# google-research/big_vision

Measured on NVIDIA H100. Metric: siglip_vit_b16_pairs_per_sec, higher is better.
Workload: dtype bf16

## Files before the change

big_vision_b200/csrc/attention.cu:

```cuda
#include "common.cuh"
#include "host_utils.h"
#include "kernels.h"

namespace bv {

namespace {

constexpr int T = 64;
constexpr int BOX_BYTES = T * 64 * 2;
constexpr float LOG2E = 1.4426950408889634f;
constexpr float LN2 = 0.6931471805599453f;
constexpr int THREADS = 128;

template <int DH>
struct Geo {
  static_assert(DH == 64 || DH == 72 || DH == 80 || DH == 96 || DH == 104, "head dims 64, 72, 80, 96, 104");
  static constexpr int TILE_BYTES = DH > 64 ? 2 * BOX_BYTES : BOX_BYTES;
  static constexpr int KSTEPS = (DH + 15) / 16;
  static_assert(KSTEPS >= 4 && KSTEPS <= 8, "one or two 64-column boxes");
  static constexpr int R = DH / 2;
  static constexpr int FWD_SMEM = 5 * TILE_BYTES + 1024 + 64;
  static constexpr int BWD_SMEM = 6 * TILE_BYTES + 1024 + 64;
};

__device__ __forceinline__ float ex2(float x) {
  float y;
  asm("ex2.approx.ftz.f32 %0, %1;" : "=f"(y) : "f"(x));
  return y;
}

int make_tmap_bnd(CUtensorMap* m, const void* ptr, int dh, int H, int64_t N, int64_t B, int64_t ld, int64_t bs) {
  if (dh == 64) {
    uint64_t dims[3] = {static_cast<uint64_t>(H) * 64, static_cast<uint64_t>(N), static_cast<uint64_t>(B)};
    uint64_t strides[2] = {static_cast<uint64_t>(ld) * 2, static_cast<uint64_t>(bs) * 2};
    uint32_t box[3] = {64, T, 1};
    return make_tmap(m, CU_TENSOR_MAP_DATA_TYPE_BFLOAT16, 3, ptr, dims, strides, box, true);
  }
  uint64_t dims[4] = {static_cast<uint64_t>(dh), static_cast<uint64_t>(H), static_cast<uint64_t>(N),
                      static_cast<uint64_t>(B)};
  uint64_t strides[3] = {static_cast<uint64_t>(dh) * 2, static_cast<uint64_t>(ld) * 2, static_cast<uint64_t>(bs) * 2};
  uint32_t box[4] = {64, 1, T, 1};
  return make_tmap(m, CU_TENSOR_MAP_DATA_TYPE_BFLOAT16, 4, ptr, dims, strides, box, true);
}

template <int DH>
__device__ __forceinline__ void load_tile(uint32_t dst, const CUtensorMap* m, uint32_t bar, int h, int row, int b) {
  if constexpr (DH == 64) {
    tma_load_3d(dst, m, bar, h * DH, row, b);
  } else {
    tma_load_4d(dst, m, bar, 0, h, row, b);
    tma_load_4d(dst + BOX_BYTES, m, bar, 64, h, row, b);
  }
}

__device__ __forceinline__ uint64_t desc_k(uint32_t tile) { return wgmma_desc_sw128(tile, 16u, 1024u); }
__device__ __forceinline__ uint64_t desc_mn(uint32_t tile) { return wgmma_desc_sw128(tile, 8192u, 1024u); }
constexpr uint64_t KSTEP_K = 32 >> 4, KSTEP_MN = 2048 >> 4;

template <int TB, int R>
__device__ __forceinline__ void wgmma_rs_dh(float (&d)[R], const uint32_t (&a)[4], uint64_t b, int scale_d) {
  if constexpr (R == 32) wgmma_rs_n64<TB>(d, a, b, scale_d);
  else if constexpr (R == 36) wgmma_rs_n72<TB>(d, a, b, scale_d);
  else if constexpr (R == 40) wgmma_rs_n80<TB>(d, a, b, scale_d);
  else if constexpr (R == 48) wgmma_rs_n96<TB>(d, a, b, scale_d);
  else wgmma_rs_n104<TB>(d, a, b, scale_d);
}

template <int DH>
__device__ __forceinline__ void mma_tile_kk(float (&d)[32], uint32_t a_tile, uint32_t b_tile) {
  const uint64_t a = desc_k(a_tile), b = desc_k(b_tile);
#pragma unroll
  for (int k = 0; k < 4; ++k) wgmma_ss_n64<0, 0>(d, a + k * KSTEP_K, b + k * KSTEP_K, k > 0 ? 1 : 0);
  if constexpr (DH > 64) {
    const uint64_t a1 = desc_k(a_tile + BOX_BYTES), b1 = desc_k(b_tile + BOX_BYTES);
#pragma unroll
    for (int k = 0; k < Geo<DH>::KSTEPS - 4; ++k) wgmma_ss_n64<0, 0>(d, a1 + k * KSTEP_K, b1 + k * KSTEP_K, 1);
  }
}
template <int R>
__device__ __forceinline__ void mma_tile_rs(float (&d)[R], const uint32_t (&p)[4][4], uint32_t b_tile) {
  const uint64_t b = desc_mn(b_tile);
#pragma unroll
  for (int k = 0; k < 4; ++k) wgmma_rs_dh<1>(d, p[k], b + k * KSTEP_MN, 1);
}

__device__ __forceinline__ void to_frags(const float (&s)[32], uint32_t (&p)[4][4]) {
#pragma unroll
  for (int kk = 0; kk < 4; ++kk) {
    p[kk][0] = pack_bf16(s[8 * kk + 0], s[8 * kk + 1]);
    p[kk][1] = pack_bf16(s[8 * kk + 2], s[8 * kk + 3]);
    p[kk][2] = pack_bf16(s[8 * kk + 4], s[8 * kk + 5]);
    p[kk][3] = pack_bf16(s[8 * kk + 6], s[8 * kk + 7]);
  }
}

template <int R>
__device__ __forceinline__ void zero(float (&d)[R]) {
#pragma unroll
  for (int i = 0; i < R; ++i) d[i] = 0.f;
}

struct FwdDev {
  int H, Nq, Nk, QT, NB;
  float scale_log2;
  float* lse;
  bf16* o;
  long long ldo, bso;
};

template <int DH>
__global__ void __launch_bounds__(THREADS)
attn_fwd_kernel(const __grid_constant__ CUtensorMap tmQ, const __grid_constant__ CUtensorMap tmK,
                const __grid_constant__ CUtensorMap tmV, const FwdDev p) {
  using G = Geo<DH>;
  constexpr int TILE_BYTES = G::TILE_BYTES;
  extern __shared__ uint8_t smem_raw[];
  const uint32_t q_s = (smem_u32(smem_raw) + 1023u) & ~1023u, k_s = q_s + TILE_BYTES, v_s = q_s + 3 * TILE_BYTES;
  const uint32_t q_bar = q_s + 5 * TILE_BYTES;
  auto kv_bar = [&](int s) { return q_bar + 8u * (1 + s); };

  const int qt = static_cast<int>(blockIdx.x % p.QT);
  const int bh = static_cast<int>(blockIdx.x / p.QT);
  const int h = bh % p.H, b = bh / p.H;
  const int tid = threadIdx.x, lane = tid & 31, warp = tid >> 5;

  auto load_kv = [&](int j) {
    const int s = j & 1;
    mbar_expect_tx(kv_bar(s), 2 * TILE_BYTES);
    load_tile<DH>(k_s + s * TILE_BYTES, &tmK, kv_bar(s), h, j * T, b);
    load_tile<DH>(v_s + s * TILE_BYTES, &tmV, kv_bar(s), h, j * T, b);
  };
  if (tid == 0) {
    mbar_init(q_bar, 1);
    mbar_init(kv_bar(0), 1);
    mbar_init(kv_bar(1), 1);
    fence_barrier_init();
    mbar_expect_tx(q_bar, TILE_BYTES);
    load_tile<DH>(q_s, &tmQ, q_bar, h, qt * T, b);
    load_kv(0);
    if (p.NB > 1) load_kv(1);
  }
  __syncthreads();

  float o[G::R], s[32];
  zero(o);
  float m[2] = {-INFINITY, -INFINITY}, l[2] = {0.f, 0.f};
  mbar_wait(q_bar, 0);
  for (int j = 0; j < p.NB; ++j) {
    const int slot = j & 1;
    mbar_wait(kv_bar(slot), (j >> 1) & 1);
    wgmma_fence();
    mma_tile_kk<DH>(s, q_s, k_s + slot * TILE_BYTES);
    wgmma_commit();
    wgmma_wait<0>();
    wgmma_fence_regs(s);
    const int kbase = j * T + 2 * (lane & 3);
    float mx[2] = {m[0], m[1]};
#pragma unroll
    for (int i = 0; i < 32; ++i) {
      const int key = kbase + 8 * (i >> 2) + (i & 1);
      s[i] = key < p.Nk ? s[i] * p.scale_log2 : -INFINITY;
      mx[(i >> 1) & 1] = fmaxf(mx[(i >> 1) & 1], s[i]);
    }
    float corr[2];
#pragma unroll
    for (int r = 0; r < 2; ++r) {
      mx[r] = fmaxf(mx[r], __shfl_xor_sync(0xffffffffu, mx[r], 1));
      mx[r] = fmaxf(mx[r], __shfl_xor_sync(0xffffffffu, mx[r], 2));
      corr[r] = ex2(m[r] - mx[r]);
      m[r] = mx[r];
      l[r] *= corr[r];
    }
#pragma unroll
    for (int i = 0; i < 32; ++i) {
      const int r = (i >> 1) & 1;
      s[i] = ex2(s[i] - m[r]);
      l[r] += s[i];
      o[i] *= corr[r];
    }
#pragma unroll
    for (int i = 32; i < G::R; ++i) o[i] *= corr[(i >> 1) & 1];
    uint32_t pf[4][4];
    to_frags(s, pf);
    wgmma_fence_regs(o);
    wgmma_fence();
    mma_tile_rs(o, pf, v_s + slot * TILE_BYTES);
    wgmma_commit();
    wgmma_wait<0>();
    wgmma_fence_regs(o);
    __syncthreads();
    if (tid == 0 && j + 2 < p.NB) load_kv(j + 2);
  }
#pragma unroll
  for (int r = 0; r < 2; ++r) {
    l[r] += __shfl_xor_sync(0xffffffffu, l[r], 1);
    l[r] += __shfl_xor_sync(0xffffffffu, l[r], 2);
  }
  const float inv[2] = {1.f / l[0], 1.f / l[1]};
#pragma unroll
  for (int r = 0; r < 2; ++r) {
    const int q = qt * T + 16 * warp + (lane >> 2) + 8 * r;
    if (q >= p.Nq) continue;
    bf16* orow = p.o + b * p.bso + static_cast<long long>(q) * p.ldo + h * DH + 2 * (lane & 3);
#pragma unroll
    for (int jj = 0; jj < DH / 8; ++jj)
      *reinterpret_cast<uint32_t*>(orow + 8 * jj) = pack_bf16(o[4 * jj + 2 * r] * inv[r], o[4 * jj + 2 * r + 1] * inv[r]);
    if ((lane & 3) == 0) p.lse[(static_cast<long long>(b) * p.H + h) * p.Nq + q] = (m[r] + __log2f(l[r])) * LN2;
  }
}

struct BwdDev {
  int H, Nq, Nk, QT, KT;
  float scale, scale_log2;
  const float* lse;
  const float* delta;
  bf16* dq; bf16* dk; bf16* dv;
  long long lddq, bsdq, lddk, bsdk, lddv, bsdv;
  float* dq_colsum; float* dk_colsum; float* dv_colsum;
};

template <int R>
__device__ __forceinline__ void tile_colsum(const float (&d)[R], float mul, int row0, int nvalid, float* colsum,
                                            int lane) {
#pragma unroll
  for (int jj = 0; jj < R / 4; ++jj) {
    float c[2] = {0.f, 0.f};
#pragma unroll
    for (int r = 0; r < 2; ++r) {
      if (row0 + 8 * r >= nvalid) continue;
      c[0] += round_bf16(d[4 * jj + 2 * r] * mul);
      c[1] += round_bf16(d[4 * jj + 2 * r + 1] * mul);
    }
#pragma unroll
    for (int e = 0; e < 2; ++e) {
      c[e] += __shfl_xor_sync(0xffffffffu, c[e], 4);
      c[e] += __shfl_xor_sync(0xffffffffu, c[e], 8);
      c[e] += __shfl_xor_sync(0xffffffffu, c[e], 16);
    }
    if (lane < 4) {
      atomicAdd(colsum + 8 * jj + 2 * lane, c[0]);
      atomicAdd(colsum + 8 * jj + 2 * lane + 1, c[1]);
    }
  }
}

template <int DH>
__global__ void __launch_bounds__(THREADS)
attn_bwd_dq_kernel(const __grid_constant__ CUtensorMap tmQ, const __grid_constant__ CUtensorMap tmK,
                   const __grid_constant__ CUtensorMap tmV, const __grid_constant__ CUtensorMap tmdO, const BwdDev p) {
  using G = Geo<DH>;
  constexpr int TILE_BYTES = G::TILE_BYTES;
  extern __shared__ uint8_t smem_raw[];
  const uint32_t q_s = (smem_u32(smem_raw) + 1023u) & ~1023u, do_s = q_s + TILE_BYTES, k_s = q_s + 2 * TILE_BYTES,
                 v_s = q_s + 4 * TILE_BYTES;
  const uint32_t q_bar = q_s + 6 * TILE_BYTES;
  auto kv_bar = [&](int s) { return q_bar + 8u * (1 + s); };

  const int qt = static_cast<int>(blockIdx.x % p.QT);
  const int bh = static_cast<int>(blockIdx.x / p.QT);
  const int h = bh % p.H, b = bh / p.H;
  const int tid = threadIdx.x, lane = tid & 31, warp = tid >> 5;

  auto load_kv = [&](int j) {
    const int s = j & 1;
    mbar_expect_tx(kv_bar(s), 2 * TILE_BYTES);
    load_tile<DH>(k_s + s * TILE_BYTES, &tmK, kv_bar(s), h, j * T, b);
    load_tile<DH>(v_s + s * TILE_BYTES, &tmV, kv_bar(s), h, j * T, b);
  };
  if (tid == 0) {
    mbar_init(q_bar, 1);
    mbar_init(kv_bar(0), 1);
    mbar_init(kv_bar(1), 1);
    fence_barrier_init();
    mbar_expect_tx(q_bar, 2 * TILE_BYTES);
    load_tile<DH>(q_s, &tmQ, q_bar, h, qt * T, b);
    load_tile<DH>(do_s, &tmdO, q_bar, h, qt * T, b);
    load_kv(0);
    if (p.KT > 1) load_kv(1);
  }
  __syncthreads();

  float dq[G::R];
  zero(dq);
  const long long bhq = (static_cast<long long>(b) * p.H + h) * p.Nq;
  const int q0 = qt * T + 16 * warp + (lane >> 2);
  float lse2[2], dl[2];
#pragma unroll
  for (int r = 0; r < 2; ++r) {
    const int q = q0 + 8 * r;
    lse2[r] = q < p.Nq ? p.lse[bhq + q] * LOG2E : INFINITY;
    dl[r] = q < p.Nq ? p.delta[bhq + q] : 0.f;
  }
  mbar_wait(q_bar, 0);
  for (int j = 0; j < p.KT; ++j) {
    const int slot = j & 1;
    mbar_wait(kv_bar(slot), (j >> 1) & 1);
    const uint32_t kj = k_s + slot * TILE_BYTES, vj = v_s + slot * TILE_BYTES;
    float s[32], dp[32];
    wgmma_fence();
    mma_tile_kk<DH>(s, q_s, kj);
    mma_tile_kk<DH>(dp, do_s, vj);
    wgmma_commit();
    wgmma_wait<0>();
    wgmma_fence_regs(s);
    wgmma_fence_regs(dp);
    const int kbase = j * T + 2 * (lane & 3);
#pragma unroll
    for (int i = 0; i < 32; ++i) {
      const int r = (i >> 1) & 1;
      const int key = kbase + 8 * (i >> 2) + (i & 1);
      const float pr = key < p.Nk ? ex2(s[i] * p.scale_log2 - lse2[r]) : 0.f;
      dp[i] = pr * (dp[i] - dl[r]);
    }
    uint32_t sf[4][4];
    to_frags(dp, sf);
    wgmma_fence_regs(dq);
    wgmma_fence();
    mma_tile_rs(dq, sf, kj);
    wgmma_commit();
    wgmma_wait<0>();
    wgmma_fence_regs(dq);
    __syncthreads();
    if (tid == 0 && j + 2 < p.KT) load_kv(j + 2);
  }
#pragma unroll
  for (int r = 0; r < 2; ++r) {
    const int q = q0 + 8 * r;
    if (q >= p.Nq) continue;
    bf16* qr = p.dq + b * p.bsdq + static_cast<long long>(q) * p.lddq + h * DH + 2 * (lane & 3);
#pragma unroll
    for (int jj = 0; jj < DH / 8; ++jj)
      *reinterpret_cast<uint32_t*>(qr + 8 * jj) = pack_bf16(dq[4 * jj + 2 * r] * p.scale, dq[4 * jj + 2 * r + 1] * p.scale);
  }
  if (p.dq_colsum != nullptr) tile_colsum(dq, p.scale, q0, p.Nq, p.dq_colsum + h * DH, lane);
}

template <int DH>
__global__ void __launch_bounds__(THREADS)
attn_bwd_dkdv_kernel(const __grid_constant__ CUtensorMap tmQ, const __grid_constant__ CUtensorMap tmK,
                     const __grid_constant__ CUtensorMap tmV, const __grid_constant__ CUtensorMap tmdO, const BwdDev p) {
  using G = Geo<DH>;
  constexpr int TILE_BYTES = G::TILE_BYTES;
  extern __shared__ uint8_t smem_raw[];
  const uint32_t k_s = (smem_u32(smem_raw) + 1023u) & ~1023u, v_s = k_s + TILE_BYTES, q_s = k_s + 2 * TILE_BYTES,
                 do_s = k_s + 4 * TILE_BYTES;
  const uint32_t kv_bar = k_s + 6 * TILE_BYTES;
  auto q_bar = [&](int s) { return kv_bar + 8u * (1 + s); };

  const int kt = static_cast<int>(blockIdx.x % p.KT);
  const int bh = static_cast<int>(blockIdx.x / p.KT);
  const int h = bh % p.H, b = bh / p.H;
  const int tid = threadIdx.x, lane = tid & 31, warp = tid >> 5;

  auto load_q = [&](int i) {
    const int s = i & 1;
    mbar_expect_tx(q_bar(s), 2 * TILE_BYTES);
    load_tile<DH>(q_s + s * TILE_BYTES, &tmQ, q_bar(s), h, i * T, b);
    load_tile<DH>(do_s + s * TILE_BYTES, &tmdO, q_bar(s), h, i * T, b);
  };
  if (tid == 0) {
    mbar_init(kv_bar, 1);
    mbar_init(q_bar(0), 1);
    mbar_init(q_bar(1), 1);
    fence_barrier_init();
    mbar_expect_tx(kv_bar, 2 * TILE_BYTES);
    load_tile<DH>(k_s, &tmK, kv_bar, h, kt * T, b);
    load_tile<DH>(v_s, &tmV, kv_bar, h, kt * T, b);
    load_q(0);
    if (p.QT > 1) load_q(1);
  }
  __syncthreads();

  float dk[G::R], dv[G::R];
  zero(dk);
  zero(dv);
  const long long bhq = (static_cast<long long>(b) * p.H + h) * p.Nq;
  const int key_row = 16 * warp + (lane >> 2);
  mbar_wait(kv_bar, 0);
  for (int i = 0; i < p.QT; ++i) {
    const int slot = i & 1;
    mbar_wait(q_bar(slot), (i >> 1) & 1);
    const uint32_t qi = q_s + slot * TILE_BYTES, doi = do_s + slot * TILE_BYTES;
    float st[32], dpt[32];
    wgmma_fence();
    mma_tile_kk<DH>(st, k_s, qi);
    mma_tile_kk<DH>(dpt, v_s, doi);
    wgmma_commit();
    float lse2[16], dl[16];
#pragma unroll
    for (int c = 0; c < 16; ++c) {
      const int q = i * T + 8 * (c >> 1) + 2 * (lane & 3) + (c & 1);
      lse2[c] = q < p.Nq ? p.lse[bhq + q] * LOG2E : INFINITY;
      dl[c] = q < p.Nq ? p.delta[bhq + q] : 0.f;
    }
    wgmma_wait<0>();
    wgmma_fence_regs(st);
    wgmma_fence_regs(dpt);
#pragma unroll
    for (int e = 0; e < 32; ++e) {
      const int c = 2 * (e >> 2) + (e & 1);
      st[e] = ex2(st[e] * p.scale_log2 - lse2[c]);
      dpt[e] = st[e] * (dpt[e] - dl[c]);
    }
    uint32_t pf[4][4], sf[4][4];
    to_frags(st, pf);
    to_frags(dpt, sf);
    wgmma_fence_regs(dv);
    wgmma_fence_regs(dk);
    wgmma_fence();
    mma_tile_rs(dv, pf, doi);
    mma_tile_rs(dk, sf, qi);
    wgmma_commit();
    wgmma_wait<0>();
    wgmma_fence_regs(dv);
    wgmma_fence_regs(dk);
    __syncthreads();
    if (tid == 0 && i + 2 < p.QT) load_q(i + 2);
  }
  const int k0 = kt * T + key_row;
#pragma unroll
  for (int r = 0; r < 2; ++r) {
    const int key = k0 + 8 * r;
    if (key >= p.Nk) continue;
    bf16* kr = p.dk + b * p.bsdk + static_cast<long long>(key) * p.lddk + h * DH + 2 * (lane & 3);
    bf16* vr = p.dv + b * p.bsdv + static_cast<long long>(key) * p.lddv + h * DH + 2 * (lane & 3);
#pragma unroll
    for (int jj = 0; jj < DH / 8; ++jj) {
      *reinterpret_cast<uint32_t*>(kr + 8 * jj) = pack_bf16(dk[4 * jj + 2 * r] * p.scale, dk[4 * jj + 2 * r + 1] * p.scale);
      *reinterpret_cast<uint32_t*>(vr + 8 * jj) = pack_bf16(dv[4 * jj + 2 * r], dv[4 * jj + 2 * r + 1]);
    }
  }
  if (p.dk_colsum != nullptr) tile_colsum(dk, p.scale, k0, p.Nk, p.dk_colsum + h * DH, lane);
  if (p.dv_colsum != nullptr) tile_colsum(dv, 1.f, k0, p.Nk, p.dv_colsum + h * DH, lane);
}

template <int DH>
__global__ void __launch_bounds__(256)
attn_delta_kernel(const bf16* __restrict__ o, const bf16* __restrict__ d_o, float* __restrict__ delta,
                  int64_t B, int H, int N, int64_t ldo, int64_t bso, int64_t lddo, int64_t bsdo) {
  constexpr int LOG2_LANES = DH == 64 ? 3 : 4, LANES = 1 << LOG2_LANES;
  const int64_t total = B * N * H;
  const int chunk = threadIdx.x & (LANES - 1);
  for (int64_t r = (blockIdx.x * static_cast<int64_t>(blockDim.x) + threadIdx.x) >> LOG2_LANES; r < total;
       r += (static_cast<int64_t>(gridDim.x) * blockDim.x) >> LOG2_LANES) {
    const int h = static_cast<int>(r % H);
    const int64_t bt = r / H;
    const int t = static_cast<int>(bt % N);
    const int64_t b = bt / N;
    float acc = 0.f;
    if (chunk < DH / 8) {
      const uint4 ao = ld_nc_na(reinterpret_cast<const uint4*>(o + b * bso + t * ldo + h * DH + chunk * 8));
      const uint4 ad = ld_nc_na(reinterpret_cast<const uint4*>(d_o + b * bsdo + t * lddo + h * DH + chunk * 8));
      acc = bf16_lo(ao.x) * bf16_lo(ad.x) + bf16_hi(ao.x) * bf16_hi(ad.x);
      acc += bf16_lo(ao.y) * bf16_lo(ad.y) + bf16_hi(ao.y) * bf16_hi(ad.y);
      acc += bf16_lo(ao.z) * bf16_lo(ad.z) + bf16_hi(ao.z) * bf16_hi(ad.z);
      acc += bf16_lo(ao.w) * bf16_lo(ad.w) + bf16_hi(ao.w) * bf16_hi(ad.w);
    }
#pragma unroll
    for (int off = 1; off < LANES; off <<= 1) acc += __shfl_xor_sync(0xffffffffu, acc, off);
    if (chunk == 0) delta[(b * H + h) * N + t] = acc;
  }
}

int check_head_dim(int head_dim, const char* who) {
  if (head_dim == 64 || head_dim == 72 || head_dim == 80 || head_dim == 96 || head_dim == 104) return BV_OK;
  set_error("%s: head_dim %d is not supported (supported head dims: 64, 72, 80, 96, 104)", who, head_dim);
  return BV_ERR_UNSUPPORTED;
}

int check_attn(const AttnArgs& a, const char* who) {
  if (a.B <= 0 || a.H <= 0 || a.Nq <= 0 || a.Nk <= 0 || a.Nq > 65536 || a.Nk > 65536) {
    set_error("%s: need 1 <= Nq,Nk <= 65536 and B,H >= 1 (got B=%lld H=%d Nq=%d Nk=%d)", who,
              (long long)a.B, a.H, a.Nq, a.Nk);
    return BV_ERR_INVALID;
  }
  const int64_t tiles = ((a.Nq > a.Nk ? a.Nq : a.Nk) + T - 1) / T;
  if (a.B * a.H * tiles > 0x7fffffffLL) {
    set_error("%s: too many (batch, head, tile) work units", who);
    return BV_ERR_INVALID;
  }
  if ((reinterpret_cast<uintptr_t>(a.o) & 15) || (a.ldo % 8) || (a.bso % 8)) {
    set_error("%s: o must be 16B aligned with strides that are multiples of 8", who);
    return BV_ERR_INVALID;
  }
  return BV_OK;
}

template <int DH>
int attention_fwd(const AttnArgs& a, cudaStream_t s) {
  using G = Geo<DH>;
  int rc = check_attn(a, "bv_attention_fwd");
  if (rc) return rc;
  FwdDev p;
  p.H = a.H; p.Nq = a.Nq; p.Nk = a.Nk;
  p.QT = (a.Nq + T - 1) / T;
  p.NB = (a.Nk + T - 1) / T;
  p.scale_log2 = a.scale * LOG2E;
  p.lse = a.lse;
  p.o = static_cast<bf16*>(a.o);
  p.ldo = a.ldo; p.bso = a.bso;
  CUtensorMap tmQ, tmK, tmV;
  if ((rc = make_tmap_bnd(&tmQ, a.q, DH, a.H, a.Nq, a.B, a.ldq, a.bsq))) return rc;
  if ((rc = make_tmap_bnd(&tmK, a.k, DH, a.H, a.Nk, a.B, a.ldk, a.bsk))) return rc;
  if ((rc = make_tmap_bnd(&tmV, a.v, DH, a.H, a.Nk, a.B, a.ldv, a.bsv))) return rc;
  const long long grid = a.B * a.H * p.QT;
  rc = check_cuda(cudaFuncSetAttribute(attn_fwd_kernel<DH>, cudaFuncAttributeMaxDynamicSharedMemorySize, G::FWD_SMEM),
                  "cudaFuncSetAttribute(attn_fwd)");
  if (rc) return rc;
  attn_fwd_kernel<DH><<<static_cast<unsigned>(grid), THREADS, G::FWD_SMEM, s>>>(tmQ, tmK, tmV, p);
  return check_cuda(cudaGetLastError(), "attn_fwd_kernel launch");
}

template <int DH>
int attention_bwd(const AttnBwdArgs& g, cudaStream_t s) {
  using G = Geo<DH>;
  const AttnArgs& a = g.f;
// ... 87 lines not shown
```

big_vision_b200/csrc/wgmma.cuh:

```cuda
#pragma once
#include <stdint.h>

namespace bv {

__device__ __forceinline__ void wgmma_fence() { asm volatile("wgmma.fence.sync.aligned;" ::: "memory"); }
__device__ __forceinline__ void wgmma_commit() { asm volatile("wgmma.commit_group.sync.aligned;" ::: "memory"); }
template <int N>
__device__ __forceinline__ void wgmma_wait() { asm volatile("wgmma.wait_group.sync.aligned %0;" ::"n"(N) : "memory"); }
template <int R>
__device__ __forceinline__ void wgmma_fence_regs(float (&d)[R]) {
#pragma unroll
  for (int i = 0; i < R; ++i) asm volatile("" : "+f"(d[i])::"memory");
}

__device__ __forceinline__ uint64_t wgmma_desc_sw128(uint32_t saddr, uint32_t lbo_bytes, uint32_t sbo_bytes) {
  uint64_t d = 0;
  d |= static_cast<uint64_t>((saddr & 0x3FFFFu) >> 4);
  d |= static_cast<uint64_t>((lbo_bytes >> 4) & 0x3FFFu) << 16;
  d |= static_cast<uint64_t>((sbo_bytes >> 4) & 0x3FFFu) << 32;
  d |= static_cast<uint64_t>(1) << 62;
  return d;
}

template <int TA, int TB>
// ... 77 lines not shown
      : "l"(a), "l"(b), "r"(scale_d), "n"(TA), "n"(TB));
}
template <int TB>
__device__ __forceinline__ void wgmma_rs_n72(float (&d)[36], const uint32_t (&a)[4], uint64_t b, int scale_d) {
  asm volatile(
      "{\n.reg .pred p;\n"
      "setp.ne.b32 p, %41, 0;\n"
      "wgmma.mma_async.sync.aligned.m64n72k16.f32.bf16.bf16 "
      "{%0, %1, %2, %3, %4, %5, %6, %7, %8, %9, %10, %11, %12, %13, %14, %15, %16, %17, %18, %19, %20, %21, %22, %23, %24, %25, %26, %27, %28, %29, %30, %31, %32, %33, %34, %35}, "
      "{%36, %37, %38, %39}, %40, p, 1, 1, %42;\n}\n"
      : "+f"(d[0]), "+f"(d[1]), "+f"(d[2]), "+f"(d[3]), "+f"(d[4]), "+f"(d[5]), "+f"(d[6]), "+f"(d[7]), "+f"(d[8]), "+f"(d[9]), "+f"(d[10]), "+f"(d[11]), "+f"(d[12]), "+f"(d[13]), "+f"(d[14]), "+f"(d[15]), "+f"(d[16]), "+f"(d[17]), "+f"(d[18]), "+f"(d[19]), "+f"(d[20]), "+f"(d[21]), "+f"(d[22]), "+f"(d[23]), "+f"(d[24]), "+f"(d[25]), "+f"(d[26]), "+f"(d[27]), "+f"(d[28]), "+f"(d[29]), "+f"(d[30]), "+f"(d[31]), "+f"(d[32]), "+f"(d[33]), "+f"(d[34]), "+f"(d[35])
      : "r"(a[0]), "r"(a[1]), "r"(a[2]), "r"(a[3]), "l"(b), "r"(scale_d), "n"(TB));
}

template <int TA, int TB>
__device__ __forceinline__ void wgmma_ss_n80(float (&d)[40], uint64_t a, uint64_t b, int scale_d) {
  asm volatile(
      "{\n.reg .pred p;\n"
      "setp.ne.b32 p, %42, 0;\n"
      "wgmma.mma_async.sync.aligned.m64n80k16.f32.bf16.bf16 "
      "{%0, %1, %2, %3, %4, %5, %6, %7, %8, %9, %10, %11, %12, %13, %14, %15, %16, %17, %18, %19, %20, %21, %22, %23, %24, %25, %26, %27, %28, %29, %30, %31, %32, %33, %34, %35, %36, %37, %38, %39}, "
      "%40, %41, p, 1, 1, %43, %44;\n}\n"
      : "+f"(d[0]), "+f"(d[1]), "+f"(d[2]), "+f"(d[3]), "+f"(d[4]), "+f"(d[5]), "+f"(d[6]), "+f"(d[7]), "+f"(d[8]), "+f"(d[9]), "+f"(d[10]), "+f"(d[11]), "+f"(d[12]), "+f"(d[13]), "+f"(d[14]), "+f"(d[15]), "+f"(d[16]), "+f"(d[17]), "+f"(d[18]), "+f"(d[19]), "+f"(d[20]), "+f"(d[21]), "+f"(d[22]), "+f"(d[23]), "+f"(d[24]), "+f"(d[25]), "+f"(d[26]), "+f"(d[27]), "+f"(d[28]), "+f"(d[29]), "+f"(d[30]), "+f"(d[31]), "+f"(d[32]), "+f"(d[33]), "+f"(d[34]), "+f"(d[35]), "+f"(d[36]), "+f"(d[37]), "+f"(d[38]), "+f"(d[39])
      : "l"(a), "l"(b), "r"(scale_d), "n"(TA), "n"(TB));
}
template <int TB>
__device__ __forceinline__ void wgmma_rs_n80(float (&d)[40], const uint32_t (&a)[4], uint64_t b, int scale_d) {
  asm volatile(
      "{\n.reg .pred p;\n"
      "setp.ne.b32 p, %45, 0;\n"
      "wgmma.mma_async.sync.aligned.m64n80k16.f32.bf16.bf16 "
      "{%0, %1, %2, %3, %4, %5, %6, %7, %8, %9, %10, %11, %12, %13, %14, %15, %16, %17, %18, %19, %20, %21, %22, %23, %24, %25, %26, %27, %28, %29, %30, %31, %32, %33, %34, %35, %36, %37, %38, %39}, "
      "{%40, %41, %42, %43}, %44, p, 1, 1, %46;\n}\n"
      : "+f"(d[0]), "+f"(d[1]), "+f"(d[2]), "+f"(d[3]), "+f"(d[4]), "+f"(d[5]), "+f"(d[6]), "+f"(d[7]), "+f"(d[8]), "+f"(d[9]), "+f"(d[10]), "+f"(d[11]), "+f"(d[12]), "+f"(d[13]), "+f"(d[14]), "+f"(d[15]), "+f"(d[16]), "+f"(d[17]), "+f"(d[18]), "+f"(d[19]), "+f"(d[20]), "+f"(d[21]), "+f"(d[22]), "+f"(d[23]), "+f"(d[24]), "+f"(d[25]), "+f"(d[26]), "+f"(d[27]), "+f"(d[28]), "+f"(d[29]), "+f"(d[30]), "+f"(d[31]), "+f"(d[32]), "+f"(d[33]), "+f"(d[34]), "+f"(d[35]), "+f"(d[36]), "+f"(d[37]), "+f"(d[38]), "+f"(d[39])
      : "r"(a[0]), "r"(a[1]), "r"(a[2]), "r"(a[3]), "l"(b), "r"(scale_d), "n"(TB));
}

template <int TA, int TB>
__device__ __forceinline__ void wgmma_ss_n96(float (&d)[48], uint64_t a, uint64_t b, int scale_d) {
  asm volatile(
      "{\n.reg .pred p;\n"
      "setp.ne.b32 p, %50, 0;\n"
      "wgmma.mma_async.sync.aligned.m64n96k16.f32.bf16.bf16 "
      "{%0, %1, %2, %3, %4, %5, %6, %7, %8, %9, %10, %11, %12, %13, %14, %15, %16, %17, %18, %19, %20, %21, %22, %23, %24, %25, %26, %27, %28, %29, %30, %31, %32, %33, %34, %35, %36, %37, %38, %39, %40, %41, %42, %43, %44, %45, %46, %47}, "
      "%48, %49, p, 1, 1, %51, %52;\n}\n"
      : "+f"(d[0]), "+f"(d[1]), "+f"(d[2]), "+f"(d[3]), "+f"(d[4]), "+f"(d[5]), "+f"(d[6]), "+f"(d[7]), "+f"(d[8]), "+f"(d[9]), "+f"(d[10]), "+f"(d[11]), "+f"(d[12]), "+f"(d[13]), "+f"(d[14]), "+f"(d[15]), "+f"(d[16]), "+f"(d[17]), "+f"(d[18]), "+f"(d[19]), "+f"(d[20]), "+f"(d[21]), "+f"(d[22]), "+f"(d[23]), "+f"(d[24]), "+f"(d[25]), "+f"(d[26]), "+f"(d[27]), "+f"(d[28]), "+f"(d[29]), "+f"(d[30]), "+f"(d[31]), "+f"(d[32]), "+f"(d[33]), "+f"(d[34]), "+f"(d[35]), "+f"(d[36]), "+f"(d[37]), "+f"(d[38]), "+f"(d[39]), "+f"(d[40]), "+f"(d[41]), "+f"(d[42]), "+f"(d[43]), "+f"(d[44]), "+f"(d[45]), "+f"(d[46]), "+f"(d[47])
      : "l"(a), "l"(b), "r"(scale_d), "n"(TA), "n"(TB));
}
template <int TB>
__device__ __forceinline__ void wgmma_rs_n96(float (&d)[48], const uint32_t (&a)[4], uint64_t b, int scale_d) {
  asm volatile(
      "{\n.reg .pred p;\n"
      "setp.ne.b32 p, %53, 0;\n"
      "wgmma.mma_async.sync.aligned.m64n96k16.f32.bf16.bf16 "
      "{%0, %1, %2, %3, %4, %5, %6, %7, %8, %9, %10, %11, %12, %13, %14, %15, %16, %17, %18, %19, %20, %21, %22, %23, %24, %25, %26, %27, %28, %29, %30, %31, %32, %33, %34, %35, %36, %37, %38, %39, %40, %41, %42, %43, %44, %45, %46, %47}, "
      "{%48, %49, %50, %51}, %52, p, 1, 1, %54;\n}\n"
      : "+f"(d[0]), "+f"(d[1]), "+f"(d[2]), "+f"(d[3]), "+f"(d[4]), "+f"(d[5]), "+f"(d[6]), "+f"(d[7]), "+f"(d[8]), "+f"(d[9]), "+f"(d[10]), "+f"(d[11]), "+f"(d[12]), "+f"(d[13]), "+f"(d[14]), "+f"(d[15]), "+f"(d[16]), "+f"(d[17]), "+f"(d[18]), "+f"(d[19]), "+f"(d[20]), "+f"(d[21]), "+f"(d[22]), "+f"(d[23]), "+f"(d[24]), "+f"(d[25]), "+f"(d[26]), "+f"(d[27]), "+f"(d[28]), "+f"(d[29]), "+f"(d[30]), "+f"(d[31]), "+f"(d[32]), "+f"(d[33]), "+f"(d[34]), "+f"(d[35]), "+f"(d[36]), "+f"(d[37]), "+f"(d[38]), "+f"(d[39]), "+f"(d[40]), "+f"(d[41]), "+f"(d[42]), "+f"(d[43]), "+f"(d[44]), "+f"(d[45]), "+f"(d[46]), "+f"(d[47])
      : "r"(a[0]), "r"(a[1]), "r"(a[2]), "r"(a[3]), "l"(b), "r"(scale_d), "n"(TB));
}

template <int TA, int TB>
__device__ __forceinline__ void wgmma_ss_n104(float (&d)[52], uint64_t a, uint64_t b, int scale_d) {
  asm volatile(
      "{\n.reg .pred p;\n"
      "setp.ne.b32 p, %54, 0;\n"
      "wgmma.mma_async.sync.aligned.m64n104k16.f32.bf16.bf16 "
      "{%0, %1, %2, %3, %4, %5, %6, %7, %8, %9, %10, %11, %12, %13, %14, %15, %16, %17, %18, %19, %20, %21, %22, %23, %24, %25, %26, %27, %28, %29, %30, %31, %32, %33, %34, %35, %36, %37, %38, %39, %40, %41, %42, %43, %44, %45, %46, %47, %48, %49, %50, %51}, "
      "%52, %53, p, 1, 1, %55, %56;\n}\n"
      : "+f"(d[0]), "+f"(d[1]), "+f"(d[2]), "+f"(d[3]), "+f"(d[4]), "+f"(d[5]), "+f"(d[6]), "+f"(d[7]), "+f"(d[8]), "+f"(d[9]), "+f"(d[10]), "+f"(d[11]), "+f"(d[12]), "+f"(d[13]), "+f"(d[14]), "+f"(d[15]), "+f"(d[16]), "+f"(d[17]), "+f"(d[18]), "+f"(d[19]), "+f"(d[20]), "+f"(d[21]), "+f"(d[22]), "+f"(d[23]), "+f"(d[24]), "+f"(d[25]), "+f"(d[26]), "+f"(d[27]), "+f"(d[28]), "+f"(d[29]), "+f"(d[30]), "+f"(d[31]), "+f"(d[32]), "+f"(d[33]), "+f"(d[34]), "+f"(d[35]), "+f"(d[36]), "+f"(d[37]), "+f"(d[38]), "+f"(d[39]), "+f"(d[40]), "+f"(d[41]), "+f"(d[42]), "+f"(d[43]), "+f"(d[44]), "+f"(d[45]), "+f"(d[46]), "+f"(d[47]), "+f"(d[48]), "+f"(d[49]), "+f"(d[50]), "+f"(d[51])
      : "l"(a), "l"(b), "r"(scale_d), "n"(TA), "n"(TB));
}
template <int TB>
__device__ __forceinline__ void wgmma_rs_n104(float (&d)[52], const uint32_t (&a)[4], uint64_t b, int scale_d) {
  asm volatile(
      "{\n.reg .pred p;\n"
      "setp.ne.b32 p, %57, 0;\n"
      "wgmma.mma_async.sync.aligned.m64n104k16.f32.bf16.bf16 "
      "{%0, %1, %2, %3, %4, %5, %6, %7, %8, %9, %10, %11, %12, %13, %14, %15, %16, %17, %18, %19, %20, %21, %22, %23, %24, %25, %26, %27, %28, %29, %30, %31, %32, %33, %34, %35, %36, %37, %38, %39, %40, %41, %42, %43, %44, %45, %46, %47, %48, %49, %50, %51}, "
      "{%52, %53, %54, %55}, %56, p, 1, 1, %58;\n}\n"
      : "+f"(d[0]), "+f"(d[1]), "+f"(d[2]), "+f"(d[3]), "+f"(d[4]), "+f"(d[5]), "+f"(d[6]), "+f"(d[7]), "+f"(d[8]), "+f"(d[9]), "+f"(d[10]), "+f"(d[11]), "+f"(d[12]), "+f"(d[13]), "+f"(d[14]), "+f"(d[15]), "+f"(d[16]), "+f"(d[17]), "+f"(d[18]), "+f"(d[19]), "+f"(d[20]), "+f"(d[21]), "+f"(d[22]), "+f"(d[23]), "+f"(d[24]), "+f"(d[25]), "+f"(d[26]), "+f"(d[27]), "+f"(d[28]), "+f"(d[29]), "+f"(d[30]), "+f"(d[31]), "+f"(d[32]), "+f"(d[33]), "+f"(d[34]), "+f"(d[35]), "+f"(d[36]), "+f"(d[37]), "+f"(d[38]), "+f"(d[39]), "+f"(d[40]), "+f"(d[41]), "+f"(d[42]), "+f"(d[43]), "+f"(d[44]), "+f"(d[45]), "+f"(d[46]), "+f"(d[47]), "+f"(d[48]), "+f"(d[49]), "+f"(d[50]), "+f"(d[51])
      : "r"(a[0]), "r"(a[1]), "r"(a[2]), "r"(a[3]), "l"(b), "r"(scale_d), "n"(TB));
}

}
```

Baseline: 2779.

## Trim wgmma width on ragged last tiles and reduce colsum atomics via shared memory

The attention forward and backward loops now choose the wgmma N width (16/32/48/64) per key or query block from how many valid rows remain, so the partial last tile of SigLIP's 196-token sequence does less matrix-multiply and softmax work. The column-sum epilogue first combines per-warp partials in shared memory, then issues one atomic per column instead of one per warp. The dK/dV kernel also gets a minBlocks launch bound of 3 for head dim 64. The cost is more template instantiations and code size, extra block-wide barriers in the epilogue, and a risk of register spilling from the occupancy bound.

```diff
diff --git a/big_vision_b200/csrc/attention.cu b/big_vision_b200/csrc/attention.cu
--- a/big_vision_b200/csrc/attention.cu
+++ b/big_vision_b200/csrc/attention.cu
@@ -66,27 +66,49 @@
   else wgmma_rs_n104<TB>(d, a, b, scale_d);
 }
 
-template <int DH>
-__device__ __forceinline__ void mma_tile_kk(float (&d)[32], uint32_t a_tile, uint32_t b_tile) {
+template <int W>
+struct Width {
+  static constexpr int value = W;
+};
+
+template <class F>
+__device__ __forceinline__ void with_block_width(int rows, F&& f) {
+  if (rows <= 16) f(Width<16>{});
+  else if (rows <= 32) f(Width<32>{});
+  else if (rows <= 48) f(Width<48>{});
+  else f(Width<64>{});
+}
+
+template <int W>
+__device__ __forceinline__ void wgmma_ss_w(float (&d)[W / 2], uint64_t a, uint64_t b, int scale_d) {
+  if constexpr (W == 16) wgmma_ss_n16<0, 0>(d, a, b, scale_d);
+  else if constexpr (W == 32) wgmma_ss_n32<0, 0>(d, a, b, scale_d);
+  else if constexpr (W == 48) wgmma_ss_n48<0, 0>(d, a, b, scale_d);
+  else wgmma_ss_n64<0, 0>(d, a, b, scale_d);
+}
+
+template <int DH, int W>
+__device__ __forceinline__ void mma_tile_kk(float (&d)[W / 2], uint32_t a_tile, uint32_t b_tile) {
   const uint64_t a = desc_k(a_tile), b = desc_k(b_tile);
 #pragma unroll
-  for (int k = 0; k < 4; ++k) wgmma_ss_n64<0, 0>(d, a + k * KSTEP_K, b + k * KSTEP_K, k > 0 ? 1 : 0);
+  for (int k = 0; k < 4; ++k) wgmma_ss_w<W>(d, a + k * KSTEP_K, b + k * KSTEP_K, k > 0 ? 1 : 0);
   if constexpr (DH > 64) {
     const uint64_t a1 = desc_k(a_tile + BOX_BYTES), b1 = desc_k(b_tile + BOX_BYTES);
 #pragma unroll
-    for (int k = 0; k < Geo<DH>::KSTEPS - 4; ++k) wgmma_ss_n64<0, 0>(d, a1 + k * KSTEP_K, b1 + k * KSTEP_K, 1);
-  }
-}
-template <int R>
-__device__ __forceinline__ void mma_tile_rs(float (&d)[R], const uint32_t (&p)[4][4], uint32_t b_tile) {
+    for (int k = 0; k < Geo<DH>::KSTEPS - 4; ++k) wgmma_ss_w<W>(d, a1 + k * KSTEP_K, b1 + k * KSTEP_K, 1);
+  }
+}
+template <int W, int R>
+__device__ __forceinline__ void mma_tile_rs(float (&d)[R], const uint32_t (&p)[W / 16][4], uint32_t b_tile) {
   const uint64_t b = desc_mn(b_tile);
 #pragma unroll
-  for (int k = 0; k < 4; ++k) wgmma_rs_dh<1>(d, p[k], b + k * KSTEP_MN, 1);
-}
-
-__device__ __forceinline__ void to_frags(const float (&s)[32], uint32_t (&p)[4][4]) {
-#pragma unroll
-  for (int kk = 0; kk < 4; ++kk) {
+  for (int k = 0; k < W / 16; ++k) wgmma_rs_dh<1>(d, p[k], b + k * KSTEP_MN, 1);
+}
+
+template <int W>
+__device__ __forceinline__ void to_frags(const float (&s)[W / 2], uint32_t (&p)[W / 16][4]) {
+#pragma unroll
+  for (int kk = 0; kk < W / 16; ++kk) {
     p[kk][0] = pack_bf16(s[8 * kk + 0], s[8 * kk + 1]);
     p[kk][1] = pack_bf16(s[8 * kk + 2], s[8 * kk + 3]);
     p[kk][2] = pack_bf16(s[8 * kk + 4], s[8 * kk + 5]);
@@ -142,22 +164,23 @@
   }
   __syncthreads();
 
-  float o[G::R], s[32];
+  float o[G::R];
   zero(o);
   float m[2] = {-INFINITY, -INFINITY}, l[2] = {0.f, 0.f};
-  mbar_wait(q_bar, 0);
-  for (int j = 0; j < p.NB; ++j) {
+  auto kv_block = [&](auto width, int j) {
+    constexpr int W = decltype(width)::value;
     const int slot = j & 1;
     mbar_wait(kv_bar(slot), (j >> 1) & 1);
+    float s[W / 2];
     wgmma_fence();
-    mma_tile_kk<DH>(s, q_s, k_s + slot * TILE_BYTES);
+    mma_tile_kk<DH, W>(s, q_s, k_s + slot * TILE_BYTES);
     wgmma_commit();
     wgmma_wait<0>();
     wgmma_fence_regs(s);
     const int kbase = j * T + 2 * (lane & 3);
     float mx[2] = {m[0], m[1]};
 #pragma unroll
-    for (int i = 0; i < 32; ++i) {
+    for (int i = 0; i < W / 2; ++i) {
       const int key = kbase + 8 * (i >> 2) + (i & 1);
       s[i] = key < p.Nk ? s[i] * p.scale_log2 : -INFINITY;
       mx[(i >> 1) & 1] = fmaxf(mx[(i >> 1) & 1], s[i]);
@@ -172,25 +195,26 @@
       l[r] *= corr[r];
     }
 #pragma unroll
-    for (int i = 0; i < 32; ++i) {
+    for (int i = 0; i < W / 2; ++i) {
       const int r = (i >> 1) & 1;
       s[i] = ex2(s[i] - m[r]);
       l[r] += s[i];
-      o[i] *= corr[r];
-    }
-#pragma unroll
-    for (int i = 32; i < G::R; ++i) o[i] *= corr[(i >> 1) & 1];
-    uint32_t pf[4][4];
-    to_frags(s, pf);
+    }
+#pragma unroll
+    for (int i = 0; i < G::R; ++i) o[i] *= corr[(i >> 1) & 1];
+    uint32_t pf[W / 16][4];
+    to_frags<W>(s, pf);
     wgmma_fence_regs(o);
     wgmma_fence();
-    mma_tile_rs(o, pf, v_s + slot * TILE_BYTES);
+    mma_tile_rs<W>(o, pf, v_s + slot * TILE_BYTES);
     wgmma_commit();
     wgmma_wait<0>();
     wgmma_fence_regs(o);
     __syncthreads();
     if (tid == 0 && j + 2 < p.NB) load_kv(j + 2);
-  }
+  };
+  mbar_wait(q_bar, 0);
+  for (int j = 0; j < p.NB; ++j) with_block_width(p.Nk - j * T, [&](auto width) { kv_block(width, j); });
 #pragma unroll
   for (int r = 0; r < 2; ++r) {
     l[r] += __shfl_xor_sync(0xffffffffu, l[r], 1);
@@ -221,7 +245,9 @@
 
 template <int R>
 __device__ __forceinline__ void tile_colsum(const float (&d)[R], float mul, int row0, int nvalid, float* colsum,
-                                            int lane) {
+                                            float* red) {
+  constexpr int DH = 2 * R;
+  const int tid = threadIdx.x, lane = tid & 31, warp = tid >> 5;
 #pragma unroll
   for (int jj = 0; jj < R / 4; ++jj) {
     float c[2] = {0.f, 0.f};
@@ -238,10 +264,14 @@
       c[e] += __shfl_xor_sync(0xffffffffu, c[e], 16);
     }
     if (lane < 4) {
-      atomicAdd(colsum + 8 * jj + 2 * lane, c[0]);
-      atomicAdd(colsum + 8 * jj + 2 * lane + 1, c[1]);
-    }
-  }
+      red[warp * DH + 8 * jj + 2 * lane] = c[0];
+      red[warp * DH + 8 * jj + 2 * lane + 1] = c[1];
+    }
+  }
+  __syncthreads();
+  for (int col = tid; col < DH; col += THREADS)
+    atomicAdd(colsum + col, (red[col] + red[DH + col]) + (red[2 * DH + col] + red[3 * DH + col]));
+  __syncthreads();
 }
 
 template <int DH>
@@ -291,38 +321,40 @@
     lse2[r] = q < p.Nq ? p.lse[bhq + q] * LOG2E : INFINITY;
     dl[r] = q < p.Nq ? p.delta[bhq + q] : 0.f;
   }
-  mbar_wait(q_bar, 0);
-  for (int j = 0; j < p.KT; ++j) {
+  auto kv_block = [&](auto width, int j) {
+    constexpr int W = decltype(width)::value;
     const int slot = j & 1;
     mbar_wait(kv_bar(slot), (j >> 1) & 1);
     const uint32_t kj = k_s + slot * TILE_BYTES, vj = v_s + slot * TILE_BYTES;
-    float s[32], dp[32];
+    float s[W / 2], dp[W / 2];
     wgmma_fence();
-    mma_tile_kk<DH>(s, q_s, kj);
-    mma_tile_kk<DH>(dp, do_s, vj);
+    mma_tile_kk<DH, W>(s, q_s, kj);
+    mma_tile_kk<DH, W>(dp, do_s, vj);
     wgmma_commit();
     wgmma_wait<0>();
     wgmma_fence_regs(s);
     wgmma_fence_regs(dp);
     const int kbase = j * T + 2 * (lane & 3);
 #pragma unroll
-    for (int i = 0; i < 32; ++i) {
+    for (int i = 0; i < W / 2; ++i) {
       const int r = (i >> 1) & 1;
       const int key = kbase + 8 * (i >> 2) + (i & 1);
       const float pr = key < p.Nk ? ex2(s[i] * p.scale_log2 - lse2[r]) : 0.f;
       dp[i] = pr * (dp[i] - dl[r]);
     }
-    uint32_t sf[4][4];
-    to_frags(dp, sf);
+    uint32_t sf[W / 16][4];
+    to_frags<W>(dp, sf);
     wgmma_fence_regs(dq);
     wgmma_fence();
-    mma_tile_rs(dq, sf, kj);
+    mma_tile_rs<W>(dq, sf, kj);
     wgmma_commit();
     wgmma_wait<0>();
     wgmma_fence_regs(dq);
     __syncthreads();
     if (tid == 0 && j + 2 < p.KT) load_kv(j + 2);
-  }
+  };
+  mbar_wait(q_bar, 0);
+  for (int j = 0; j < p.KT; ++j) with_block_width(p.Nk - j * T, [&](auto width) { kv_block(width, j); });
 #pragma unroll
   for (int r = 0; r < 2; ++r) {
     const int q = q0 + 8 * r;
@@ -332,11 +364,12 @@
     for (int jj = 0; jj < DH / 8; ++jj)
       *reinterpret_cast<uint32_t*>(qr + 8 * jj) = pack_bf16(dq[4 * jj + 2 * r] * p.scale, dq[4 * jj + 2 * r + 1] * p.scale);
   }
-  if (p.dq_colsum != nullptr) tile_colsum(dq, p.scale, q0, p.Nq, p.dq_colsum + h * DH, lane);
-}
-
-template <int DH>
-__global__ void __launch_bounds__(THREADS)
+  float* red = reinterpret_cast<float*>(smem_raw + (k_s - smem_u32(smem_raw)));
+  if (p.dq_colsum != nullptr) tile_colsum(dq, p.scale, q0, p.Nq, p.dq_colsum + h * DH, red);
+}
+
+template <int DH>
+__global__ void __launch_bounds__(THREADS, DH == 64 ? 3 : 1)
 attn_bwd_dkdv_kernel(const __grid_constant__ CUtensorMap tmQ, const __grid_constant__ CUtensorMap tmK,
                      const __grid_constant__ CUtensorMap tmV, const __grid_constant__ CUtensorMap tmdO, const BwdDev p) {
   using G = Geo<DH>;
@@ -376,19 +409,19 @@
   zero(dv);
   const long long bhq = (static_cast<long long>(b) * p.H + h) * p.Nq;
   const int key_row = 16 * warp + (lane >> 2);
-  mbar_wait(kv_bar, 0);
-  for (int i = 0; i < p.QT; ++i) {
+  auto q_block = [&](auto width, int i) {
+    constexpr int W = decltype(width)::value;
     const int slot = i & 1;
     mbar_wait(q_bar(slot), (i >> 1) & 1);
     const uint32_t qi = q_s + slot * TILE_BYTES, doi = do_s + slot * TILE_BYTES;
-    float st[32], dpt[32];
+    float st[W / 2], dpt[W / 2];
     wgmma_fence();
-    mma_tile_kk<DH>(st, k_s, qi);
-    mma_tile_kk<DH>(dpt, v_s, doi);
+    mma_tile_kk<DH, W>(st, k_s, qi);
+    mma_tile_kk<DH, W>(dpt, v_s, doi);
     wgmma_commit();
-    float lse2[16], dl[16];
-#pragma unroll
-    for (int c = 0; c < 16; ++c) {
+    float lse2[W / 4], dl[W / 4];
+#pragma unroll
+    for (int c = 0; c < W / 4; ++c) {
       const int q = i * T + 8 * (c >> 1) + 2 * (lane & 3) + (c & 1);
       lse2[c] = q < p.Nq ? p.lse[bhq + q] * LOG2E : INFINITY;
       dl[c] = q < p.Nq ? p.delta[bhq + q] : 0.f;
@@ -397,26 +430,28 @@
     wgmma_fence_regs(st);
     wgmma_fence_regs(dpt);
 #pragma unroll
-    for (int e = 0; e < 32; ++e) {
+    for (int e = 0; e < W / 2; ++e) {
       const int c = 2 * (e >> 2) + (e & 1);
       st[e] = ex2(st[e] * p.scale_log2 - lse2[c]);
       dpt[e] = st[e] * (dpt[e] - dl[c]);
     }
-    uint32_t pf[4][4], sf[4][4];
-    to_frags(st, pf);
-    to_frags(dpt, sf);
+    uint32_t pf[W / 16][4], sf[W / 16][4];
+    to_frags<W>(st, pf);
+    to_frags<W>(dpt, sf);
     wgmma_fence_regs(dv);
     wgmma_fence_regs(dk);
     wgmma_fence();
-    mma_tile_rs(dv, pf, doi);
-    mma_tile_rs(dk, sf, qi);
+    mma_tile_rs<W>(dv, pf, doi);
+    mma_tile_rs<W>(dk, sf, qi);
     wgmma_commit();
     wgmma_wait<0>();
     wgmma_fence_regs(dv);
     wgmma_fence_regs(dk);
     __syncthreads();
     if (tid == 0 && i + 2 < p.QT) load_q(i + 2);
-  }
+  };
+  mbar_wait(kv_bar, 0);
+  for (int i = 0; i < p.QT; ++i) with_block_width(p.Nq - i * T, [&](auto width) { q_block(width, i); });
   const int k0 = kt * T + key_row;
 #pragma unroll
   for (int r = 0; r < 2; ++r) {
@@ -430,8 +465,9 @@
       *reinterpret_cast<uint32_t*>(vr + 8 * jj) = pack_bf16(dv[4 * jj + 2 * r], dv[4 * jj + 2 * r + 1]);
     }
   }
-  if (p.dk_colsum != nullptr) tile_colsum(dk, p.scale, k0, p.Nk, p.dk_colsum + h * DH, lane);
-  if (p.dv_colsum != nullptr) tile_colsum(dv, 1.f, k0, p.Nk, p.dv_colsum + h * DH, lane);
+  float* red = reinterpret_cast<float*>(smem_raw + (q_s - smem_u32(smem_raw)));
+  if (p.dk_colsum != nullptr) tile_colsum(dk, p.scale, k0, p.Nk, p.dk_colsum + h * DH, red);
+  if (p.dv_colsum != nullptr) tile_colsum(dv, 1.f, k0, p.Nk, p.dv_colsum + h * DH, red);
 }
 
 template <int DH>
diff --git a/big_vision_b200/csrc/wgmma.cuh b/big_vision_b200/csrc/wgmma.cuh
--- a/big_vision_b200/csrc/wgmma.cuh
+++ b/big_vision_b200/csrc/wgmma.cuh
@@ -183,4 +183,40 @@
       : "r"(a[0]), "r"(a[1]), "r"(a[2]), "r"(a[3]), "l"(b), "r"(scale_d), "n"(TB));
 }
 
-}
+template <int TA, int TB>
+__device__ __forceinline__ void wgmma_ss_n16(float (&d)[8], uint64_t a, uint64_t b, int scale_d) {
+  asm volatile(
+      "{\n.reg .pred p;\n"
+      "setp.ne.b32 p, %10, 0;\n"
+      "wgmma.mma_async.sync.aligned.m64n16k16.f32.bf16.bf16 "
+      "{%0, %1, %2, %3, %4, %5, %6, %7}, "
+      "%8, %9, p, 1, 1, %11, %12;\n}\n"
+      : "+f"(d[0]), "+f"(d[1]), "+f"(d[2]), "+f"(d[3]), "+f"(d[4]), "+f"(d[5]), "+f"(d[6]), "+f"(d[7])
+      : "l"(a), "l"(b), "r"(scale_d), "n"(TA), "n"(TB));
+}
+
+template <int TA, int TB>
+__device__ __forceinline__ void wgmma_ss_n32(float (&d)[16], uint64_t a, uint64_t b, int scale_d) {
+  asm volatile(
+      "{\n.reg .pred p;\n"
+      "setp.ne.b32 p, %18, 0;\n"
+      "wgmma.mma_async.sync.aligned.m64n32k16.f32.bf16.bf16 "
+      "{%0, %1, %2, %3, %4, %5, %6, %7, %8, %9, %10, %11, %12, %13, %14, %15}, "
+      "%16, %17, p, 1, 1, %19, %20;\n}\n"
+      : "+f"(d[0]), "+f"(d[1]), "+f"(d[2]), "+f"(d[3]), "+f"(d[4]), "+f"(d[5]), "+f"(d[6]), "+f"(d[7]), "+f"(d[8]), "+f"(d[9]), "+f"(d[10]), "+f"(d[11]), "+f"(d[12]), "+f"(d[13]), "+f"(d[14]), "+f"(d[15])
+      : "l"(a), "l"(b), "r"(scale_d), "n"(TA), "n"(TB));
+}
+
+template <int TA, int TB>
+__device__ __forceinline__ void wgmma_ss_n48(float (&d)[24], uint64_t a, uint64_t b, int scale_d) {
+  asm volatile(
+      "{\n.reg .pred p;\n"
+      "setp.ne.b32 p, %26, 0;\n"
+      "wgmma.mma_async.sync.aligned.m64n48k16.f32.bf16.bf16 "
+      "{%0, %1, %2, %3, %4, %5, %6, %7, %8, %9, %10, %11, %12, %13, %14, %15, %16, %17, %18, %19, %20, %21, %22, %23}, "
+      "%24, %25, p, 1, 1, %27, %28;\n}\n"
+      : "+f"(d[0]), "+f"(d[1]), "+f"(d[2]), "+f"(d[3]), "+f"(d[4]), "+f"(d[5]), "+f"(d[6]), "+f"(d[7]), "+f"(d[8]), "+f"(d[9]), "+f"(d[10]), "+f"(d[11]), "+f"(d[12]), "+f"(d[13]), "+f"(d[14]), "+f"(d[15]), "+f"(d[16]), "+f"(d[17]), "+f"(d[18]), "+f"(d[19]), "+f"(d[20]), "+f"(d[21]), "+f"(d[22]), "+f"(d[23])
+      : "l"(a), "l"(b), "r"(scale_d), "n"(TA), "n"(TB));
+}
+
+}
```

Result: no change. 2806, median of 6 (+1.0%).
